# sebhaan/geobo

Hardware: AMD Instinct MI355X
Metric: voxels/sec posterior (mean+var) for 64^3 x 2-prop joint inversion; fp64 roofline % (higher is better)
Workload: dtype f64

## Files before the change

### geobo_amd/_lib.py

```python
import ctypes as C
import os

LIB_PATH = os.environ.get("GEOBO_HIP_LIB") or os.path.join(os.path.dirname(os.path.abspath(__file__)), "lib", "libgeobo_hip.so")

_dp = C.c_void_p
_i64 = C.c_int64
_f64 = C.c_double
_int = C.c_int
_sz = C.c_size_t

SIGNATURES = {
    "geobo_version": (_int, []),
    "geobo_pad_m": (_i64, [_i64]),
    "geobo_pad_n": (_i64, [_i64]),
    "geobo_k_block": (_int, [_int, _dp, _dp, _dp, _i64, _dp, _dp, _dp, _i64, _f64, _f64, _f64, _f64, _dp, _i64, _dp]),
    "geobo_k_block_f32": (_int, [_int, _dp, _dp, _dp, _i64, _dp, _dp, _dp, _i64, _f64, _f64, _f64, _f64, _dp, _i64, _dp]),
    "geobo_k_block_grid": (_int, [_int, _int, _int, _dp, _dp, _i64, _i64, _i64, _i64, _int, _dp, _i64, _dp]),
    "geobo_lattice_wbuild": (_int, [_i64, _int, _int, _int, _dp, _dp, _dp, _dp]),
    "geobo_lattice_wplanes": (_int, [_i64, _int, _int, _int, _dp, _dp, _dp, _dp]),
    "geobo_xz2d_fold_inv_strided": (_int, [_int, _i64, _int, _dp, _i64, _i64, _dp, _dp, _dp, _i64, _i64, _i64, _dp]),
    "geobo_xz2d_fold_inv_mul": (_int, [_int, _i64, _int, _dp, _i64, _dp, _i64, _dp, _dp, _dp, _i64, _i64, _i64, _dp]),
    "geobo_xz2d_fold_conv_fwd": (_int, [_int, _i64, _int, _dp, _i64, _dp, _i64, _dp, _i64, _dp, _dp, _dp, _i64, _i64, _dp]),
    "geobo_sumsq_accum": (_int, [_i64, _i64, _dp, _i64, _dp, _i64, _int, _dp, _i64, _dp]),
    "geobo_lamdot_z": (_int, [_i64, _int, _int, _int, _dp, _dp, _dp, _dp]),
    "geobo_centro_fill": (_int, [_dp, _i64, _i64, _i64, _dp]),
    "geobo_transpose": (_int, [_i64, _i64, _dp, _i64, _dp, _i64, _dp]),
    "geobo_mirror_rows": (_int, [_dp, _i64, _i64, _i64, _i64, _int, _dp]),
    "geobo_mirror_dev_ws_bytes": (_sz, []),
    "geobo_mirror_dev": (_int, [_dp, _i64, _dp, _i64, _i64, _int, _int, _dp, _dp, _sz, _dp]),
    "geobo_colgemv_ws_bytes": (_sz, [_i64, _i64]),
    "geobo_colgemv": (_int, [_i64, _i64, _dp, _i64, _dp, _dp, _dp, _sz, _dp]),
    "geobo_rowgemv": (_int, [_i64, _i64, _dp, _i64, _dp, _dp, _dp]),
    "geobo_convert": (_int, [_int, _dp, _i64, _dp, _i64, _i64, _i64, _dp]),
    "geobo_round_f32": (_int, [_dp, _i64, _dp]),
    "geobo_k_eval": (_int, [_int, _dp, _i64, _f64, _f64, _f64, _f64, _dp, _dp]),
    "geobo_a_sens": (_int, [_int, C.POINTER(_f64), _dp, _i64, _int, _int, _int, _dp, _dp, _dp, _f64, _f64, _dp, _i64, _dp]),
    "geobo_a_sens_slab": (_int, [_int, C.POINTER(_f64), _dp, _i64, _int, _int, _int, _dp, _dp, _dp, _f64, _f64, _int, _int, _dp, _i64, _i64, _dp]),
    "geobo_potential": (_int, [_int, C.POINTER(_f64), _dp, _dp, _dp, _i64, _dp, _dp]),
    "geobo_ak_fused": (_int, [_int, _dp, _i64, _i64, _i64, _dp, _dp, _dp, _i64, _i64, _f64, _f64, _f64, _f64, _dp, _i64, _dp]),
    "geobo_ak_points": (_int, [_int, _dp, _i64, _i64, _i64, _dp, _dp, _dp, _dp, _dp, _dp, _i64, _f64, _f64, _f64, _f64, _dp, _i64, _dp]),
    "geobo_cov_table": (_int, [_int, _int, _int, _int, _f64, _f64, _f64, _f64, _f64, _f64, _f64, _dp, _dp]),
    "geobo_ak_fused_grid": (_int, [_dp, _i64, _i64, _i64, _int, _int, _int, _dp, _i64, _i64, _dp, _i64, _dp]),
    "geobo_gemm_nt": (_int, [_i64, _i64, _i64, _f64, _dp, _i64, _dp, _i64, _f64, _dp, _i64, _int, _i64, _dp]),
    "geobo_tile_order": (_i64, [_int, _int, _int, _int, _int, _int, _int, C.POINTER(_int), _i64]),
    "geobo_gemm_map": (_int, [_int, _int, _int, _int, _int, _int, _int, _int, C.POINTER(_int)]),
    "geobo_gemm_nt_splitk": (_int, [_i64, _i64, _i64, _int, _dp, _i64, _dp, _i64, _dp, _i64, _int, _i64, _dp, _sz, _dp]),
    "geobo_gemm_nn": (_int, [_i64, _i64, _i64, _f64, _dp, _i64, _dp, _i64, _f64, _dp, _i64, _int, _int, _dp]),
    "geobo_gemm_batched": (_int, [_int, _i64, _i64, _i64, _f64, _dp, _i64, _i64, _dp, _i64, _i64, _f64, _dp, _i64, _i64, _i64, _i64, _int, _dp]),
    "geobo_gemm_fold_lamdot": (_int, [_i64, _i64, _i64, _dp, _i64, _dp, _i64, _i64, _dp, _int, _i64, _dp, _i64, _dp]),
    "geobo_gemm_fold": (_int, [_int, _int, _i64, _i64, _i64, _dp, _i64, _i64, _dp, _i64, _i64, _dp, _i64, _i64, _i64, _i64, _i64, _dp]),
# ... 111 lines not shown
```

### geobo_amd/csrc/reduce.hip

```cpp
#include <hip/hip_runtime.h>
#include <stdint.h>
#include "geobo_hip.h"

namespace {

typedef double v2d __attribute__((ext_vector_type(2)));

__global__ void __launch_bounds__(256) sumsq_accum_kernel(int64_t rows, int64_t n2, const double* __restrict__ a, int64_t lda,
                                                          const double* __restrict__ b, int64_t ldb, int slots, double* __restrict__ ss,
                                                          int64_t ld_ss) {
  const int64_t c2 = (int64_t)blockIdx.x * 256 + threadIdx.x;
  if (c2 >= n2) return;
  const int slot = blockIdx.y;
  v2d acc = *reinterpret_cast<const v2d*>(ss + slot * ld_ss + 2 * c2);
  if (b) {
    for (int64_t r = slot; r < rows; r += slots) {
      const v2d x = *reinterpret_cast<const v2d*>(a + r * lda + 2 * c2) + *reinterpret_cast<const v2d*>(b + r * ldb + 2 * c2);
      acc.x = __builtin_fma(x.x, x.x, acc.x);
      acc.y = __builtin_fma(x.y, x.y, acc.y);
    }
  } else {
    for (int64_t r = slot; r < rows; r += slots) {
      const v2d x = *reinterpret_cast<const v2d*>(a + r * lda + 2 * c2);
      acc.x = __builtin_fma(x.x, x.x, acc.x);
// ... 57 lines not shown
        v2d w;
        w.x = v.y;
        w.y = v.x;
        *reinterpret_cast<v2d*>(dst + (n - 2 - c)) = w;
      } else {
        dst[n - 2 - c] = v.y;
        dst[n - 1 - c] = v.x;
      }
    } else {
      dst[0] = src[c];
    }
  }
}

__global__ void __launch_bounds__(256) mirror_rows_kernel(double* __restrict__ X, int64_t ld, int64_t m, int64_t r0, int64_t nb, int nz2) {
  const int64_t e = (int64_t)blockIdx.x * 256 + threadIdx.x;
  if (e >= nb * nz2) return;
  const int64_t b = e / nz2;
  const int64_t se = (nb - 1 - b) * nz2 + (e - b * nz2);
  for (int64_t r = r0 + blockIdx.y; r < m; r += gridDim.y)
    reinterpret_cast<v2d*>(X + r * ld)[e] = reinterpret_cast<const v2d*>(X + (m - 1 - r) * ld)[se];
}

__device__ __forceinline__ double max_keep_nan(double m, double v) { return (v > m || v != v) ? v : m; }

constexpr int MIRROR_SLOTS_X = 4, MIRROR_SLOTS_Y = 256;

__global__ void __launch_bounds__(256) mirror_dev_kernel(const double* __restrict__ a, int64_t lda, const double* __restrict__ b, int64_t ldb,
                                                         int64_t rows, int nx, int nz2, double* __restrict__ part) {
  __shared__ double sh[2][4];
  double dev = 0.0, mx = 0.0;
  const int pairs = nx * nz2;
  for (int64_t r = blockIdx.y; r < rows; r += gridDim.y) {
    const v2d* pa = reinterpret_cast<const v2d*>(a + r * lda);
    const v2d* pb = reinterpret_cast<const v2d*>(b + (rows - 1 - r) * ldb);
    for (int e = blockIdx.x * 256 + threadIdx.x; e < pairs; e += gridDim.x * 256) {
      const int x = e / nz2;
      const v2d u = pa[e], w = pb[(nx - 1 - x) * nz2 + (e - x * nz2)];
      dev = max_keep_nan(max_keep_nan(dev, __builtin_fabs(u.x - w.x)), __builtin_fabs(u.y - w.y));
      mx = max_keep_nan(max_keep_nan(mx, __builtin_fabs(u.x)), __builtin_fabs(u.y));
      mx = max_keep_nan(max_keep_nan(mx, __builtin_fabs(w.x)), __builtin_fabs(w.y));
    }
  }
  for (int o = 32; o > 0; o >>= 1) {
    dev = max_keep_nan(dev, __shfl_xor(dev, o));
    mx = max_keep_nan(mx, __shfl_xor(mx, o));
// ... 54 lines not shown
                     rows, cols, src, lds, dst, ldd);
  return hipGetLastError() == hipSuccess ? GEOBO_OK : GEOBO_E_LAUNCH;
}

extern "C" int geobo_centro_fill(double* B, int64_t ld, int64_t n, int64_t r0, void* stream) {
  if (!B || ((uintptr_t)B & 15) || n < 0 || r0 < 0 || r0 > n || 2 * r0 < n || ld < n) return GEOBO_E_ARG;
  if (ld & 1) return GEOBO_E_ALIGN;
  if (r0 == n) return GEOBO_OK;
  const int64_t gy = n - r0 < 65535 ? n - r0 : 65535;
  hipLaunchKernelGGL(centro_fill_kernel, dim3((unsigned)(((n + 1) / 2 + 255) / 256), (unsigned)gy), dim3(256), 0, (hipStream_t)stream, B, ld, n, r0);
  return hipGetLastError() == hipSuccess ? GEOBO_OK : GEOBO_E_LAUNCH;
}

extern "C" int geobo_mirror_rows(double* X, int64_t ld, int64_t m, int64_t r0, int64_t nb, int nz, void* stream) {
  if (!X || m < 0 || r0 < 0 || r0 > m || 2 * r0 < m || nb <= 0 || nz <= 0 || nb * nz > ld) return GEOBO_E_ARG;
  if ((nz & 1) || (ld & 1) || ((uintptr_t)X & 15)) return GEOBO_E_ALIGN;
  if (r0 == m) return GEOBO_OK;
  const int64_t pairs = nb * (nz / 2), gy = m - r0 < 65535 ? m - r0 : 65535;
  hipLaunchKernelGGL(mirror_rows_kernel, dim3((unsigned)((pairs + 255) / 256), (unsigned)gy), dim3(256), 0, (hipStream_t)stream, X, ld, m, r0, nb,
                     nz / 2);
  return hipGetLastError() == hipSuccess ? GEOBO_OK : GEOBO_E_LAUNCH;
}

extern "C" size_t geobo_mirror_dev_ws_bytes(void) { return sizeof(double) * 2 * MIRROR_SLOTS_X * MIRROR_SLOTS_Y; }

extern "C" int geobo_mirror_dev(const double* a, int64_t lda, const double* b, int64_t ldb, int64_t rows, int nx, int nz, double* out2, void* ws,
                                size_t ws_bytes, void* stream) {
  if (!a || !b || !out2 || !ws || rows <= 0 || nx <= 0 || nz <= 0 || ws_bytes < geobo_mirror_dev_ws_bytes()) return GEOBO_E_ARG;
  if ((int64_t)nx * nz > lda || (int64_t)nx * nz > ldb || (int64_t)nx * nz >= (1LL << 31)) return GEOBO_E_ARG;
  if ((nz & 1) || (lda & 1) || (ldb & 1) || ((uintptr_t)a & 15) || ((uintptr_t)b & 15) || ((uintptr_t)ws & 15)) return GEOBO_E_ALIGN;
  const int pairs = nx * (nz / 2);
  const int gx = (pairs + 255) / 256 < MIRROR_SLOTS_X ? (pairs + 255) / 256 : MIRROR_SLOTS_X;
  const int gy = rows < MIRROR_SLOTS_Y ? (int)rows : MIRROR_SLOTS_Y;
  hipLaunchKernelGGL(mirror_dev_kernel, dim3(gx, gy), dim3(256), 0, (hipStream_t)stream, a, lda, b, ldb, rows, nx, nz / 2, (double*)ws);
  hipLaunchKernelGGL(mirror_dev_finish_kernel, dim3(1), dim3(256), 0, (hipStream_t)stream, (const double*)ws, gx * gy, out2);
  return hipGetLastError() == hipSuccess ? GEOBO_OK : GEOBO_E_LAUNCH;
}

extern "C" int geobo_rowgemv(int64_t m, int64_t n, const double* X, int64_t ld, const double* v, double* out, void* stream) {
  if (!X || !v || !out) return GEOBO_E_ARG;
  if (m <= 0 || n <= 0) return GEOBO_OK;
  if ((n & 1) || (ld & 1) || ld < n || ((uintptr_t)X & 15) || ((uintptr_t)v & 15)) return GEOBO_E_ALIGN;
  const int64_t nb = m < 256 * 16 ? m : 256 * 16;
  hipLaunchKernelGGL(rowgemv_kernel, dim3((unsigned)nb), dim3(256), 0, (hipStream_t)stream, m, n / 2, X, ld, v, out);
  return hipGetLastError() == hipSuccess ? GEOBO_OK : GEOBO_E_LAUNCH;
}
// ... 27 lines not shown
```

### geobo_amd/engine.py

```python
import math
import os
import time

import numpy as np
import torch

from . import geometry, hip
from .plan import COLUMN_FORM_MAX_BYTES, engine_options, feed_options, gram_gx_route, plan_route
from .columnform import ColumnExchangeMixin
from .rowform import RowFormMixin
from .operators import StreamedOperator
from .transposed import TransposedPosteriorMixin
from .information import SetStatisticsMixin
from .crossval import CrossValidationMixin
from .blocksupport import BlockSupportMixin
from .pointpred import PointPredictionMixin
from .resources import ResourceMixin
from .geobodies import GeobodyMixin
from .intercepts import InterceptMixin
from .append import AppendRowsMixin
from .reweight import ReweightMixin
from .step import Prior, Step
from .sharding import (EmulatedGroup, allreduce_sum_, assemble_columns, backend_of, exchange_blocks, exchange_blocks_finish,
                       exchange_blocks_start, gather_rows, gather_slices, shard_columns)

F64 = hip.F64


class _GramFeed:

    def __init__(self, gram, lams, S, store_all=True):
# ... 103 lines not shown
        s = settings
        self.nx, self.ny, self.nz = int(s.xNcube), int(s.yNcube), int(s.zNcube)
        self.N = self.nx * self.ny * self.nz
        self.N_pad = hip.pad_n(self.N)
        self.Ms = self.nx * self.ny
        self.Ms_pad = hip.pad_m(self.Ms)
        self.c0, self.c1 = shard_columns(self.N_pad, world, rank)
        self.nc = self.c1 - self.c0
        self._xyz = None
        self._A = {}
        self._ws = {}
        self._host = {}
        self._auto_denied = set()
        self._pending_exchange = None
        self.use_grid = self.nz >= 16 and self.nz % 2 == 0
        if method not in ("auto", "dense", "spectral"):
            raise ValueError("method must be 'auto', 'dense' or 'spectral'")
        self.method = method
        env = os.environ
        self.route = plan_route(self.nx, self.ny, self.nz, world=world, rank=rank, assembly=assembly, operators=operators, method=method,
                                env=env)
        self.options = engine_options(env)
        self.feed = feed_options(env)
        self.use_spectral = self.route.spectral
        if method == "spectral" and not self.use_spectral:
            raise ValueError("spectral method needs grid extents % 16 == 0 and column shards on y-slab boundaries")
        if self.route.operators == "streamed":
            self.streamed = True
        if self.route.note and self.N >= 32768:
            import warnings
            warnings.warn("geobo_amd route %s: %s" % (self.route.describe(), self.route.note), RuntimeWarning, stacklevel=3)
        self._spectral = None
        self._lattice_plan = None
        self._gram, self._lam, self._edgeV = None, {}, {}
        self._lamW, self._edgeVt = {}, {}
        self.aka_mirror_on = self.options.aka_mirror
        self.aka_mirror, self._mirror, self._mirror_meas = {}, {}, None
        self.z_spectrum_on = self.options.z_spectrum
        self.rows_static = self.route.rows
        self.exchange = self.route.exchange
        self._deny = {}
        self.step_route = None
        self._step = None
        self.last = None
        if self.streamed and not self.use_spectral:
            raise ValueError("streamed operators feed the spectral product: needs the spectral method's grid conditions")
# ... 357 lines not shown
                    hip.convert(out64, out)
            if Md:
                self._cov_rows(step.prior, 2, j, sel_t, self.c0, AK[off_d:off_d + Md, cols])
        return AK

    def _cov_rows(self, prior, i, j, rows_t, col0, out):
        ncv = min(out.shape[1], max(self.N - col0, 0))
        if ncv <= 0:
            return out
        if self.use_grid and col0 % 2 == 0:
            tab = prior.table(self, i, j)
            return hip.k_block_grid(tab, self.nx, self.ny, self.nz, rows_t, col0, out[:, :ncv])
        xyz = self.grid_points()
        rows = tuple(c[rows_t] for c in xyz)
        colc = tuple(c[col0:col0 + out.shape[1]] for c in xyz)
        return prior.k_block(self, i, j, rows, colc, out)

    def _assemble_AK_spectral(self, step, AK, A_g, A_m):
        sp, nc, props = self._spectral_product(), self.nc, step.props
        plane = self.nx * self.nz
        y0, y1 = self.c0 // plane, self.c1 // plane
        if self.exchange:
            return self._assemble_AK_spectral_exchange(step, AK)
        for s_, A in ((0, A_g), (1, A_m)):
            lams, outs, blocks = [], [], []
            for jj, j in enumerate(props):
                gen = sp.eigenvalues(step.prior.table(self, s_, j))
                step.gens[(s_, j)] = gen
                if step.sym and (s_, j) not in ((0, 0), (0, 1), (1, 1)):
                    continue
                lams.append(gen)
                blocks.append(j)
                outs.append(AK[s_ * self.Ms_pad:s_ * self.Ms_pad + self.Ms, jj * nc:(jj + 1) * nc])
            pooled = (isinstance(A, StreamedOperator) and A.lattice is not None and A.lattice.jy is not None and not self.f32
                      and sp.pool_applies())
            Mrun = step.mirror if (s_ == 1 and step.mirror) else self.Ms
            fl = sp.flops(Mrun, len(lams), y1 - y0, fwd_planes=sp.pool_planes(Mrun) if pooled else None)
            fv = sp.flops_valu(Mrun, len(lams), y1 - y0)
            feed = self._gram_feed(step, s_, blocks) if (y0, y1) == (0, self.ny) else None
            if feed is not None:
                fl += self._gram.flops_gx(Mrun * len(lams))

            def product_rows(gx, A=A, lams=lams, outs=outs, Mrun=Mrun, pooled=pooled):
                if not self.f32 and not isinstance(A, StreamedOperator):
                    return sp.product(A, Mrun, lams, [o[:Mrun] for o in outs], y0, y1, gx=gx)
                Rb = sp.R
                abuf = self._op_rows_buffer() if isinstance(A, StreamedOperator) else None
                scr = [self._workspace2d("ak_rows64_%d" % jj, Rb, nc) for jj in range(len(lams))] if self.f32 else None
                pool = sp.plane_pool(A.lattice, Mrun, A.lattice.jy, A.lattice.jx) if pooled else None
                for r0 in range(0, Mrun, Rb):
                    R = min(Rb, Mrun - r0)
                    if pool is not None:
                        src = pool.rows(r0)
                    elif abuf is not None and A.lattice is not None:
                        src = A.lattice.rows(r0)
                    else:
                        src = A.rows_into(abuf, r0, R) if abuf is not None else A[r0:r0 + R]
                    dst = [b[:R] for b in scr] if scr is not None else [o[r0:r0 + R] for o in outs]
                    sp.product(src, R, lams, dst, y0, y1, gx=gx and gx.at(r0))
                    if scr is not None:
                        for jj in range(len(lams)):
                            hip.convert(dst[jj], outs[jj][r0:r0 + R])
            self._timed("spectral_product", fl, lambda: product_rows(feed), valu=fv)
            if feed is not None and not feed.store_all:
                step.ak_fill.append(lambda fill=product_rows: fill(None))

    def _gram_feed(self, step, s_, blocks):
        gram, sp = self._gram, self._spectral_product()
        funcs = ("grav", "magn")
        if not (gram_gx_route(self.feed, self.route.family, step.sym, self.f32, self.world, self.exchange, self.nx, self.ny, self.nz, sp.forms)
                and gram is not None and gram.gx_applies() and sp.gx_applies() and all(j in (0, 1) and self._lam.get(funcs[j]) is not None for j in blocks)):
            return None
        S = [self._workspace("gram_S_%d%d" % (s_, j), (self.Ms * gram.Py * gram.Px,)) for j in blocks]
        for j, Sj in zip(blocks, S):
            step.gram_S[(s_, j)] = Sj
        return _GramFeed(gram, [self._lam[funcs[j]][1] for j in blocks], S, store_all=False)

    def _edge_spectrum(self, func, k, ycols):
        key = (func, k)
        hit = self._edgeV.get(key)
        if hit is None or hit[0] != ycols.data_ptr():
            hit = self._edgeV[key] = (ycols.data_ptr(), self._gram.edge_eigen(ycols))
        return hit[1]

    MIRROR_BOUND = 2.0 ** -48

    def _mirror_static(self, plan):
        return bool(self.aka_mirror_on and plan is not None and plan["rowmajor"] and self.route.family == "single" and self.world == 1
# ... 181 lines not shown
                    jj = props.index(j)
                    out[j * N:(j + 1) * N] = h[(k * P_c + jj) * N:(k * P_c + jj + 1) * N]
                else:
                    out[j * N:(j + 1) * N] = np.nan
            outs.append(out)
        return outs

    @_on_device
    def posterior(self, A_g, A_m, sel, y_g, y_m, y_d, lengths, crossweights, kernelfunc, gp_sigma, gp_amp=1.0,
                  props=(0, 1, 2), calclogl=True, want_mean_var=True, keep_K=False, potrf_schedule=None):
        props = tuple(props)
        assert 0 in props and 1 in props, "gravity and magnetic blocks are needed for AkA"
        sel = np.asarray(sel, dtype=np.int64)
        sel_t = torch.as_tensor(sel, device=self.device) if sel.size else None
        t = self._tick("start")
        scales = self._step_row_scale(sel)
        y = self._pad_y(y_g, y_m, y_d, hip.pad_m(2 * self.Ms_pad + len(sel)), None if scales is None else scales[1])
        if self.rows_static and not self._rows_denied and not self._rows_ok(A_g, A_m) and all(f in self._op_args for f in ("grav", "magn")):
            A_g, A_m = (self.operator(f, *self._op_args[f][:1], B=self._op_args[f][1], axes=self._op_args[f][2]) for f in ("grav", "magn"))
        step = self._step = self._new_step(Prior(kernelfunc, lengths, weight_matrix(crossweights), gp_amp), props, sel_t, gp_sigma,
                                           keep_signal=bool(keep_K), row_scale=scales, sym=not self.rows_static and self._sym_ok(A_g, A_m))
        M_pad = step.M_pad
        step.mirror = self._mirror_rows(step, A_m)
        for f, rec in self.aka_mirror.items():
            rec["taken"] = bool(f == "magn" and step.mirror)
        AK = self._assemble_AK(step, A_g, A_m)
        self.step_route = "rows" if step.rowpath else ("single" if step.sym else "columns")
        t = self._tick("ak_fused", t)
        AkA = self._assemble_AkA(step, AK, A_g, A_m)
        if self.aka_hook is not None:
            self.aka_hook(AkA)
        t = self._tick("aka", t)
        if self._potrf_ctx is None:
            self._potrf_ctx = hip.PotrfContext()
        Linv, info = self._timed("potrf_inv", 2.0 * M_pad ** 3 / 3.0, lambda: hip.potrf_inv(
            AkA, self._workspace("Linv", (M_pad, M_pad)), self._workspace("potrf_ws", (hip.potrf_ws_doubles(M_pad),)),
            ctx=self._potrf_ctx, schedule=potrf_schedule or self.options.potrf), alg=(2 * self.Ms + len(sel)) ** 3 * 2.0 / 3.0)
        L = AkA
        if scales is not None and scales[1].size:
            Linv.diagonal()[torch.as_tensor(scales[1], device=self.device)] = 0.0
        self._finish_exchange()
        u, stats = hip.trmv_stats(Linv, y, L)
        t = self._tick("cholesky", t)
        out = dict(info=0, M_pad=M_pad, lengths=[float(v) for v in lengths])

        def check_factor():
# ... 52 lines not shown
                    ws = self._workspace("post_ws", (hip.posterior_ws_doubles(M_pad, pw),))
                    parts = [hip.posterior_reduce(Linv, self._panel64("post_panel64", AK[:, cs:min(ncols, cs + pw)], cols=pw), u,
                                                  gp_amp * 1.0, ws, m_valid=Mv) for cs in range(0, ncols, pw)]
                    return torch.cat([p[0] for p in parts]), torch.cat([p[1] for p in parts])
                mu_l, var_l = self._timed("posterior_reduce", fl, panels, alg=(1.0 * Mu * Mu + 4.0 * Mu) * nv)
            one = self.world == 1 and self.N == self.N_pad
            mv = (mu_l, var_l, self.nc) if self.world == 1 else None
            N_ = len(props) * self.N
            hq = self._to_host_async(torch.cat([mu_l.reshape(-1)[:N_], var_l.reshape(-1)[:N_]]), 0) if one else None
            check_factor()
            t = self._tick("posterior", t)
            if one:
                out["mu"], out["var"] = self._results_to_host(mu_l, var_l, props, queued=hq)
            else:
                mu = assemble_columns(gather_slices(mu_l, len(props), self.N_pad, self.world, self.group), props, self.N,
                                      self.N_pad, self.world, to_host=self._to_host)
                var = assemble_columns(gather_slices(var_l, len(props), self.N_pad, self.world, self.group), props, self.N,
                                       self.N_pad, self.world, to_host=self._to_host)
                out["mu"], out["var"] = mu, var
            self._tick("d2h", t)
        whole = AK is not None and not step.sym
        self.last = _LastStep(L=L, Linv=Linv, u=u, AK=AK if whole else None, AK_partial=None if whole else AK, AK_complete=whole, props=props,
                              sel=sel, ops=(A_g, A_m), step=step, mv=mv, uu=out.get("uu"), logdet=out.get("logdet"))
        fills = list(step.ak_fill)
        if step.mirror and step.mirror < self.Ms:
            jj, nc, Msp, Mm = props.index(1), self.nc, self.Ms_pad, step.mirror
            fills.append(lambda: hip.mirror_rows(AK[Msp:Msp + self.Ms, jj * nc:jj * nc + self.N], self.Ms, Mm, self.nx * self.ny, self.nz))
        self.last.complete = _LastStep.chain(fills)
        return out

    def _derivative_gram(self, A_g, A_m, sel_t, prior, slot):
        step = self._new_step(prior, (0, 1, 2), sel_t, None, ak_slot="dK_AK", aka_slot=slot,
                              sym=not self.rows_static and self._sym_ok(A_g, A_m))
        return self._assemble_AkA(step, self._assemble_AK(step, A_g, A_m), A_g, A_m)

    @_on_device
    def logl_grad(self, A_g, A_m, sel, y_g, y_m, y_d, lengths, crossweights, kernelfunc, gp_sigma, gp_amp, directions,
                  potrf_schedule=None):
        if self.world > 1:
            raise ValueError("logl_grad runs on one rank (world = %d): the multi-rank gradient is not implemented" % self.world)
        if self.f32:
            raise ValueError("logl_grad needs the fp64 assembly (assembly='f32' keeps fp32 covariance tables)")
        directions = [np.asarray(d, dtype=float).reshape(3) for d in directions]
        if len(directions) > 3:
            raise ValueError("at most three length directions per evaluation")
        props = (0, 1, 2)
        r = self.posterior(A_g, A_m, sel, y_g, y_m, y_d, lengths, crossweights, kernelfunc, gp_sigma, gp_amp=gp_amp, props=props,
                           calclogl=True, want_mean_var=False, keep_K=True, potrf_schedule=potrf_schedule)
        W = weight_matrix(crossweights)
        Linv, u = self.last["Linv"], self.last["u"]
        M_pad = Linv.shape[0]
        sel = np.asarray(sel, dtype=np.int64)
# ... 115 lines not shown
```

### geobo_amd/hip.py

```python
import ctypes as C

import numpy as np
import torch

from . import _lib

F64 = torch.float64

KERNEL_IDS = {"d2": 0, "exp": 1, "exp_x": 2, "matern32": 3, "matern32_x": 4, "sparse": 5, "sparse_x": 6,
              "exp_dl": 7, "exp_x_dl1": 8, "exp_x_dl2": 9, "matern32_dl": 10, "matern32_x_dl1": 11, "matern32_x_dl2": 12,
              "sparse_dl": 13, "sparse_x_dl1": 14, "sparse_x_dl2": 15}
FUNC_IDS = {"grav": 0, "magn": 1}
from .plan import (PAD_M, PAD_N, SPECTRAL_AXIS_N, SPECTRAL_Y3T_NY, SPECTRAL_Y_NY, TOEPLITZ_ADD_NY, TOEPLITZ_NY, TOEPLITZ_Y2T_NY,
                   XZ2D_FOLD_N, XZ2D_SHAPES, YMUL_SHAPES)


def kernel_id(name, cross, deriv=None):
    if name not in ("exp", "matern32", "sparse"):
        raise ValueError("unknown kernelfunc %r (expected 'sparse', 'exp' or 'matern32')" % (name,))
    if deriv is None:
        return KERNEL_IDS[name + ("_x" if cross else "")]
    if isinstance(deriv, bool) or deriv not in (1, 2):
        raise ValueError("deriv must be None, 1 or 2, got %r" % (deriv,))
    if not cross:
# ... 173 lines not shown
def centro_fill(B, n, r0):
    lib = require_gpu()
    ld = _rowmajor(B, "B")
    assert B.shape[0] >= n and B.shape[1] >= n
    _lib.check(lib.geobo_centro_fill(_p(B), int(ld), int(n), int(r0), _stream()), "geobo_centro_fill")
    return B


def transpose(src, dst):
    lib = require_gpu()
    lds, ldd = _rowmajor(src, "src"), _rowmajor(dst, "dst")
    rows, cols = src.shape
    assert dst.shape[0] >= cols and dst.shape[1] >= rows
    _lib.check(lib.geobo_transpose(int(rows), int(cols), _p(src), int(lds), _p(dst), int(ldd), _stream()), "geobo_transpose")
    return dst


def mirror_rows(X, m, r0, nb, nz):
    lib = require_gpu()
    ld = _rowmajor(X, "X")
    assert X.shape[0] >= m and X.shape[1] >= nb * nz
    _lib.check(lib.geobo_mirror_rows(_p(X), int(ld), int(m), int(r0), int(nb), int(nz), _stream()), "geobo_mirror_rows")
    return X


def mirror_dev_ws_doubles():
    return require_gpu().geobo_mirror_dev_ws_bytes() // 8


def mirror_dev(a, b, rows, nx, nz, out=None, ws=None):
    lib = require_gpu()
    lda, ldb = _rowmajor(a, "a"), _rowmajor(b, "b")
    assert a.shape[0] >= rows and b.shape[0] >= rows
    nws = lib.geobo_mirror_dev_ws_bytes() // 8
    if ws is None:
        ws = torch.empty(nws, dtype=F64, device=a.device)
    if out is None:
        out = torch.empty(2, dtype=F64, device=a.device)
    _lib.check(lib.geobo_mirror_dev(_p(a), int(lda), _p(b), int(ldb), int(rows), int(nx), int(nz), _p(_chk(out, "out")), _p(_chk(ws, "ws")),
                                    ws.numel() * 8, _stream()), "geobo_mirror_dev")
    return out


def convert(src, dst):
    lib = require_gpu()
    assert src.shape == dst.shape and src.dim() == 2 and src.stride(1) == 1 and dst.stride(1) == 1
# ... 1073 lines not shown
```

### geobo_amd/plan.py

```python
from dataclasses import asdict, dataclass, make_dataclass

PAD_M, PAD_N = 256, 128
XZ2D_SHAPES = ((48, 64), (64, 64), (64, 32))
XZ2D_FOLD_N = (64,)
TOEPLITZ_NY = (16, 32, 48, 64, 80, 96, 112, 128)
SPECTRAL_AXIS_N = (80, 96, 112, 128)
SPECTRAL_Y_NY = (32, 48, 64, 80, 96, 112, 128)
TOEPLITZ_Y2T_NY = (32, 48, 64)
TOEPLITZ_ADD_NY = (80, 96, 112, 128)
SPECTRAL_Y3T_NY = (80, 96, 112, 128)
YMUL_SHAPES = ((128, 64),)
INTEGER_BASIS_N = (32, 64)
ROWS_MIN_VOXELS = 1 << 18
ROWS_MIN_PLANE = 96 * 96
ROWS_MIN_VOXELS_MID, ROWS_MIN_PLANE_MID = 3 << 17, 64 * 64
COLUMN_FORM_MAX_BYTES = 160 << 30
ROWS_MIN_VOXELS_FUSED = 1 << 17


SWITCHES = {"fused_xz": "GEOBO_SPECTRAL_FUSED_XZ",
            "fold": "GEOBO_XZ_FOLD",
            "quad": "GEOBO_XZ_QUAD",
            "dense_y": "GEOBO_SPECTRAL_DENSE_Y",
            "y_mfma": "GEOBO_Y_MFMA",
# ... 19 lines not shown
                  "row_chunk": ("GEOBO_ROW_CHUNK", 0, int),
                  "potrf": ("GEOBO_POTRF", "auto", lambda v: "dag" if v[:1] == "d" else "streams")}
EngineOptions = make_dataclass("EngineOptions", [(k, type(d)) for k, (_, d, _p) in ENGINE_OPTIONS.items()], frozen=True)


def engine_options(env=None):
    env = {} if env is None else env
    return EngineOptions(**{k: parse(env[var]) if var in env else default for k, (var, default, parse) in ENGINE_OPTIONS.items()})


FEED_OPTIONS = {"gram_gx": ("GEOBO_GRAM_GX", True, _on)}
FeedOptions = make_dataclass("FeedOptions", [(k, type(d)) for k, (_, d, _p) in FEED_OPTIONS.items()], frozen=True)


def feed_options(env=None):
    env = {} if env is None else env
    return FeedOptions(**{k: parse(env[var]) if var in env else default for k, (var, default, parse) in FEED_OPTIONS.items()})


def gram_gx_route(opts, family, sym, f32, world, exchange, nx, ny, nz, forms):
    return bool(opts.gram_gx and sym and family == "single" and not f32 and world == 1 and not exchange
                and nx == 64 and nz == 64 and ny % 2 == 0 and 4 <= ny <= 64
                and forms.xz == "fold" and forms.gram_x == "fold" and forms.y != "spectrum")


def half_integer(n):
    return n not in INTEGER_BASIS_N


@dataclass(frozen=True)
class Forms:
    xz: str
    x_axis4: bool
    y: str
    y_two_term: str
    y3t: bool
    y2s: bool
    fold: bool
    ss: str
    lattice_feed: bool
    plane_yx: str
    gram_x: str
    gram_y_axis4: bool
    zx: bool
    z_mul: bool
    ymul_slabs: tuple
# ... 137 lines not shown
```

### geobo_amd/step.py

```python
from dataclasses import dataclass, field


class Prior:

    def __init__(self, name, lengths, W, amp, deriv=None):
        self.name, self.lengths, self.W, self.amp = name, lengths, W, amp
        self.deriv = None if deriv is None else [float(v) for v in deriv]

    def terms(self, i, j):
        from .hip import kernel_id
        w, d = self.W[i][j], self.deriv
        if d is None:
            return [(kernel_id(self.name, i != j), w)]
        if i == j:
            return [(kernel_id(self.name, False, 1), w * d[j])]
        return [(kernel_id(self.name, True, 1), w * d[j]), (kernel_id(self.name, True, 2), w * d[i])]

    def table(self, eng, i, j):
        tabs = [eng._cov_table(kid, self.lengths[j], self.lengths[i], w, self.amp) for kid, w in self.terms(i, j)]
        for t in tabs[1:]:
            tabs[0].add_(t)
        return tabs[0]

    def k_block(self, eng, i, j, rows, cols, out):
# ... 23 lines not shown
        hip.ak_points(terms[0][0], A, xyz, q_xyz, self.lengths[j], self.lengths[s], terms[0][1], self.amp, out)
        for kid, w in terms[1:]:
            tmp = eng._workspace2d("dak_points_tmp", out.shape[0], out.shape[1])
            hip.ak_points(kid, A, xyz, q_xyz, self.lengths[j], self.lengths[s], w, self.amp, tmp)
            out.add_(tmp)
        return out


@dataclass
class Step:
    prior: Prior
    props: tuple
    sel_t: object
    Md: int
    M_pad: int
    noise: object = None
    ak_slot: str = "AK"
    aka_slot: str = "AkA"
    keep_signal: bool = False
    row_scale: object = None
    sym: bool = False
    rowpath: bool = False
    mirror: int = 0
    gens: dict = field(default_factory=dict)
    fullrows: dict = field(default_factory=dict)
    gram_S: dict = field(default_factory=dict)
    ak_fill: list = field(default_factory=list)
```

### geobo_amd/transposed.py

```python

import torch

from . import hip
from .operators import StreamedOperator

F64 = hip.F64


class TransposedPosteriorMixin:
    def _sym_ok(self, A_g, A_m):
        if not self._zpath_static_ok():
            return False
        return (self._gram is not None and self._gram.edge_supported() and self.Ms_pad == self.nx * self.ny
                and all(self._lam.get(f) is not None and self._lam[f][0] is A for f, A in (("grav", A_g), ("magn", A_m))))

    def _assemble_AkA_sym(self, step, AkA, AK, A_g, A_m):
        gram, pl, ny, Msp, nc = self._gram, self.nx * self.nz, self.ny, self.Ms_pad, self.nc
        Md, off_d, props = step.Md, 2 * self.Ms_pad, step.props
        lam = {0: self._lam["grav"][1], 1: self._lam["magn"][1]}
        ops = {0: A_g, 1: A_m}

        def edge_cols(sp_, k, iy):
            A = ops[sp_]
            if isinstance(A, StreamedOperator):
                return A.edge[:, k * pl:(k + 1) * pl] if A.lattice is not None else A.slab_into(self._workspace2d("op_slab", Msp, pl), iy, iy + 1)
            return A[:, iy * pl:(iy + 1) * pl]

        def rows_times_AT(X, nrows, sp_, out, S=None):
            if S is not None:
                gram.back_rows(S, nrows, out)
            else:
                gram.gram_rows(X, nrows, lam[sp_], out, 0, ny)
            for k, iy in enumerate((0, ny - 1)):
                gram.edge_rows(X[:, iy * pl:], nrows, self._edge_spectrum(("grav", "magn")[sp_], k, edge_cols(sp_, k, iy)), out)
        blk = lambda r0, j: AK[r0:, props.index(j) * nc:(props.index(j) + 1) * nc]

        Mm = step.mirror or self.Ms

        def run():
            rows_times_AT(blk(0, 0), self.Ms, 0, AkA[0:, 0:Msp], S.get((0, 0)))
            rows_times_AT(blk(0, 1), self.Ms, 1, AkA[0:, Msp:2 * Msp], S.get((0, 1)))
            rows_times_AT(blk(Msp, 1), Mm, 1, AkA[Msp:, Msp:2 * Msp], S.get((1, 1)))
            hip.transpose(AkA[:Msp, Msp:2 * Msp], AkA[Msp:2 * Msp, :Msp])
            if Md:
                rows_times_AT(blk(off_d, 0), Md, 0, AkA[off_d:, 0:Msp])
                rows_times_AT(blk(off_d, 1), Md, 1, AkA[off_d:, Msp:2 * Msp])
        S = step.gram_S
        nfed = sum(self.Ms if s_ == 0 else Mm for s_, _ in S)
        self._timed("aka_lattice", gram.flops(2 * self.Ms + Mm + 2 * Md - nfed, ny) + gram.flops_back(nfed), run)
        if step.mirror:
            self._timed("aka_centro_fill", 0.0, lambda: hip.centro_fill(AkA[Msp:Msp + self.Ms, Msp:Msp + self.Ms], self.Ms, (self.Ms + 1) // 2))
        return self._finish_AkA(step, AkA)

    def _zpath_static_ok(self):
        if not self.route.single or self.exchange:
            return False
        self._spectral_product()
        return True

    def _zpath_ok(self, step, AK):
        return (self._zpath_static_ok() and AK is not None and AK.dtype == F64
                and all((s_, j) in step.gens for s_ in (0, 1) for j in step.props))

    def _resident_operator(self, A, func):
        if not isinstance(A, StreamedOperator):
            return A
        R = self._workspace2d("A_" + func, self.Ms_pad, self.N_pad)
        xed, yed, zed = A.axes_dev
        hip.a_sens(A.func, A.Bv, A.locd, self.nx, self.ny, self.nz, xed, yed, zed, A.mul, A.div, R, plan=A.plan, ws=A.lws)
        return R

    def _lattice_Z(self, Lview, nrows, func, A, out, zx=False, edge=None):
# ... 199 lines not shown
```

### include/geobo_hip.h

```cpp
#ifndef GEOBO_HIP_H
#define GEOBO_HIP_H

#include <stddef.h>
#include <stdint.h>

#ifdef __cplusplus
extern "C" {
#endif

#define GEOBO_VERSION 213


#define GEOBO_PAD_M 256
#define GEOBO_PAD_N 128

enum { GEOBO_OK = 0, GEOBO_E_ARG = -1, GEOBO_E_ALIGN = -2, GEOBO_E_LAUNCH = -3, GEOBO_E_UNSUPPORTED = -4 };

enum {
  GEOBO_K_D2 = 0,
  GEOBO_K_EXP = 1,
  GEOBO_K_EXP_X = 2,
  GEOBO_K_MATERN32 = 3,
  GEOBO_K_MATERN32_X = 4,
  GEOBO_K_SPARSE = 5,
// ... 177 lines not shown
int geobo_spectral_y3t(int ny, int64_t C, int64_t plane, int64_t R, int nprop, const double* in_g, const double* in_m,
                       const double* const* tabs_g, const double* const* tabs_m, double* const* outs, const double* basis, void* stream);

int geobo_spectral_axis(int inverse, int n, int64_t C, int64_t plane_in, int64_t plane_out, int64_t item_in, int64_t item_out, int64_t items,
                        const double* in, double* out, const double* basis, int mask_ends, void* stream);

enum { GEOBO_POTRF_AUTO = 0, GEOBO_POTRF_STREAMS = 1, GEOBO_POTRF_DAG = 2 };
size_t geobo_potrf_ws_bytes(int64_t m);
int geobo_potrf_ctx_create(void** ctx);
int geobo_potrf_ctx_destroy(void* ctx);
int geobo_potrf_inv(int64_t m, double* A, int64_t ld, double* Linv, int64_t ldi, int* info, void* ws,
                    size_t ws_bytes, void* ctx, int schedule, void* stream);

int geobo_rowgemv(int64_t m, int64_t n, const double* X, int64_t ld, const double* v, double* out, void* stream);

int geobo_sumsq_accum(int64_t rows, int64_t n, const double* a, int64_t lda, const double* b, int64_t ldb, int slots, double* ss,
                      int64_t ld_ss, void* stream);

int geobo_lamdot_z(int64_t batch, int planes, int px, int nz, const double* D, const double* lam, double* out, void* stream);

int geobo_centro_fill(double* B, int64_t ld, int64_t n, int64_t r0, void* stream);
int geobo_transpose(int64_t rows, int64_t cols, const double* src, int64_t lds, double* dst, int64_t ldd, void* stream);
int geobo_mirror_rows(double* X, int64_t ld, int64_t m, int64_t r0, int64_t nb, int nz, void* stream);
size_t geobo_mirror_dev_ws_bytes(void);
int geobo_mirror_dev(const double* a, int64_t lda, const double* b, int64_t ldb, int64_t rows, int nx, int nz, double* out2, void* ws,
                     size_t ws_bytes, void* stream);

size_t geobo_posterior_ws_bytes(int64_t m, int64_t ncols);
int geobo_posterior_reduce(int64_t m, int64_t ncols, const double* Linv, int64_t ldi, const double* AK, int64_t ldak,
                           const double* u, double prior_var, double* mu, double* var, int64_t m_valid, void* ws,
                           size_t ws_bytes, void* stream);

size_t geobo_kinv_dot_ws_bytes(int64_t m, int T);
int geobo_kinv_dot(int64_t m, const double* Linv, int64_t ldl, const double* alpha, int T, const double* const* G, int64_t ldg,
                   const int64_t* seg, double* out, void* ws, size_t ws_bytes, void* stream);

int geobo_trmv_stats(int64_t m, const double* Linv, int64_t ldi, const double* y, const double* L, int64_t ld,
                     double* u, double* stats, void* stream);

int geobo_mfma_f64_peak(int blocks, int iters, double* out, void* stream);

int geobo_mfma_mix(int mode, int nv, int blocks, int iters, double* out, void* stream);

enum { GEOBO_RNG_PRIOR = 0, GEOBO_RNG_OBS = 1 };
#define GEOBO_FFT_INVERSE 1
#define GEOBO_FFT_IN_PAIRS 2
// ... 80 lines not shown
```

Measured before the change: 2.501 million.

## Compute grav-magn cross Gram block from mirrored magn rows instead of grav rows

Adds a route that computes the off-diagonal AK·Aᵀ cross block from the magnetic side. Only the mirror half of rows (Mm) goes through the interior Gram, and centro-symmetric fill, plane mirroring and a transpose complete the block. The AK products for the cross blocks the symmetric path needs are reorganised to match, and leftover blocks are deferred to the late fill. This replaces a full Ms-row Gram with an Mm-row one plus cheap copy kernels. It adds a new mirror_planes kernel and complexity around which AK blocks are filled when. It is enabled by default for 64³ grids.

```diff
diff --git a/geobo_amd/_lib.py b/geobo_amd/_lib.py
--- a/geobo_amd/_lib.py
+++ b/geobo_amd/_lib.py
@@ -26,6 +26,7 @@
     "geobo_centro_fill": (_int, [_dp, _i64, _i64, _i64, _dp]),
     "geobo_transpose": (_int, [_i64, _i64, _dp, _i64, _dp, _i64, _dp]),
     "geobo_mirror_rows": (_int, [_dp, _i64, _i64, _i64, _i64, _int, _dp]),
+    "geobo_mirror_planes": (_int, [_dp, _i64, _dp, _i64, _i64, _i64, _i64, _int, _int, _dp]),
     "geobo_mirror_dev_ws_bytes": (_sz, []),
     "geobo_mirror_dev": (_int, [_dp, _i64, _dp, _i64, _i64, _int, _int, _dp, _dp, _sz, _dp]),
     "geobo_colgemv_ws_bytes": (_sz, [_i64, _i64]),
diff --git a/geobo_amd/csrc/reduce.hip b/geobo_amd/csrc/reduce.hip
--- a/geobo_amd/csrc/reduce.hip
+++ b/geobo_amd/csrc/reduce.hip
@@ -103,6 +103,16 @@
     reinterpret_cast<v2d*>(X + r * ld)[e] = reinterpret_cast<const v2d*>(X + (m - 1 - r) * ld)[se];
 }
 
+__global__ void __launch_bounds__(256) mirror_planes_kernel(const double* __restrict__ src, int64_t lds, double* __restrict__ dst, int64_t ldd,
+                                                            int64_t m, int64_t r0, int64_t r1, int nx, int nz2) {
+  const int64_t e = (int64_t)blockIdx.x * 256 + threadIdx.x;
+  if (e >= (int64_t)nx * nz2) return;
+  const int64_t x = e / nz2;
+  const int64_t se = (nx - 1 - x) * nz2 + (e - x * nz2);
+  for (int64_t r = r0 + blockIdx.y; r < r1; r += gridDim.y)
+    reinterpret_cast<v2d*>(dst + (m - 1 - r) * ldd)[e] = reinterpret_cast<const v2d*>(src + r * lds)[se];
+}
+
 __device__ __forceinline__ double max_keep_nan(double m, double v) { return (v > m || v != v) ? v : m; }
 
 constexpr int MIRROR_SLOTS_X = 4, MIRROR_SLOTS_Y = 256;
@@ -203,6 +213,18 @@
   return hipGetLastError() == hipSuccess ? GEOBO_OK : GEOBO_E_LAUNCH;
 }
 
+extern "C" int geobo_mirror_planes(const double* src, int64_t lds, double* dst, int64_t ldd, int64_t m, int64_t r0, int64_t r1, int nx, int nz,
+                                   void* stream) {
+  if (!src || !dst || m < 0 || r0 < 0 || r0 > r1 || r1 > m || nx <= 0 || nz <= 0 || (int64_t)nx * nz > lds || (int64_t)nx * nz > ldd)
+    return GEOBO_E_ARG;
+  if ((nz & 1) || (lds & 1) || (ldd & 1) || ((uintptr_t)src & 15) || ((uintptr_t)dst & 15)) return GEOBO_E_ALIGN;
+  if (r0 == r1) return GEOBO_OK;
+  const int64_t pairs = (int64_t)nx * (nz / 2), gy = r1 - r0 < 65535 ? r1 - r0 : 65535;
+  hipLaunchKernelGGL(mirror_planes_kernel, dim3((unsigned)((pairs + 255) / 256), (unsigned)gy), dim3(256), 0, (hipStream_t)stream, src, lds, dst,
+                     ldd, m, r0, r1, nx, nz / 2);
+  return hipGetLastError() == hipSuccess ? GEOBO_OK : GEOBO_E_LAUNCH;
+}
+
 extern "C" size_t geobo_mirror_dev_ws_bytes(void) { return sizeof(double) * 2 * MIRROR_SLOTS_X * MIRROR_SLOTS_Y; }
 
 extern "C" int geobo_mirror_dev(const double* a, int64_t lda, const double* b, int64_t ldb, int64_t rows, int nx, int nz, double* out2, void* ws,
diff --git a/geobo_amd/engine.py b/geobo_amd/engine.py
--- a/geobo_amd/engine.py
+++ b/geobo_amd/engine.py
@@ -6,7 +6,7 @@
 import torch
 
 from . import geometry, hip
-from .plan import COLUMN_FORM_MAX_BYTES, engine_options, feed_options, gram_gx_route, plan_route
+from .plan import COLUMN_FORM_MAX_BYTES, cross_options, cross_rows_route, engine_options, feed_options, gram_gx_route, plan_route
 from .columnform import ColumnExchangeMixin
 from .rowform import RowFormMixin
 from .operators import StreamedOperator
@@ -156,6 +156,7 @@
                                 env=env)
         self.options = engine_options(env)
         self.feed = feed_options(env)
+        self.cross = cross_options(env)
         self.use_spectral = self.route.spectral
         if method == "spectral" and not self.use_spectral:
             raise ValueError("spectral method needs grid extents % 16 == 0 and column shards on y-slab boundaries")
@@ -559,16 +560,16 @@
         y0, y1 = self.c0 // plane, self.c1 // plane
         if self.exchange:
             return self._assemble_AK_spectral_exchange(step, AK)
+        kept = ((0, 0), (0, 1), (1, 1))
+        run = ((0, 0), (1, 0), (1, 1)) if step.cross_rows == "magn" else kept
         for s_, A in ((0, A_g), (1, A_m)):
-            lams, outs, blocks = [], [], []
+            gen_of, out_of = {}, {}
             for jj, j in enumerate(props):
-                gen = sp.eigenvalues(step.prior.table(self, s_, j))
-                step.gens[(s_, j)] = gen
-                if step.sym and (s_, j) not in ((0, 0), (0, 1), (1, 1)):
-                    continue
-                lams.append(gen)
-                blocks.append(j)
-                outs.append(AK[s_ * self.Ms_pad:s_ * self.Ms_pad + self.Ms, jj * nc:(jj + 1) * nc])
+                gen_of[j] = sp.eigenvalues(step.prior.table(self, s_, j))
+                step.gens[(s_, j)] = gen_of[j]
+                out_of[j] = AK[s_ * self.Ms_pad:s_ * self.Ms_pad + self.Ms, jj * nc:(jj + 1) * nc]
+            blocks = [j for j in props if not step.sym or (s_, j) in run]
+            lams, outs = [gen_of[j] for j in blocks], [out_of[j] for j in blocks]
             pooled = (isinstance(A, StreamedOperator) and A.lattice is not None and A.lattice.jy is not None and not self.f32
                       and sp.pool_applies())
             Mrun = step.mirror if (s_ == 1 and step.mirror) else self.Ms
@@ -599,8 +600,11 @@
                         for jj in range(len(lams)):
                             hip.convert(dst[jj], outs[jj][r0:r0 + R])
             self._timed("spectral_product", fl, lambda: product_rows(feed), valu=fv)
-            if feed is not None and not feed.store_all:
-                step.ak_fill.append(lambda fill=product_rows: fill(None))
+            whole = feed is None or feed.store_all
+            late = [j for j in props if (not step.sym or (s_, j) in kept) and not (whole and j in blocks)]
+            if late:
+                step.ak_fill.append(lambda fill=product_rows, lams=[gen_of[j] for j in late], outs=[out_of[j] for j in late]:
+                                    fill(None, lams=lams, outs=outs))
 
     def _gram_feed(self, step, s_, blocks):
         gram, sp = self._gram, self._spectral_product()
@@ -828,6 +832,7 @@
                                            keep_signal=bool(keep_K), row_scale=scales, sym=not self.rows_static and self._sym_ok(A_g, A_m))
         M_pad = step.M_pad
         step.mirror = self._mirror_rows(step, A_m)
+        step.cross_rows = "magn" if cross_rows_route(self.cross, step.sym, step.mirror, self.nx, self.ny, self.nz) else "grav"
         for f, rec in self.aka_mirror.items():
             rec["taken"] = bool(f == "magn" and step.mirror)
         AK = self._assemble_AK(step, A_g, A_m)
@@ -926,12 +931,15 @@
         whole = AK is not None and not step.sym
         self.last = _LastStep(L=L, Linv=Linv, u=u, AK=AK if whole else None, AK_partial=None if whole else AK, AK_complete=whole, props=props,
                               sel=sel, ops=(A_g, A_m), step=step, mv=mv, uu=out.get("uu"), logdet=out.get("logdet"))
+        self.last.complete = self._ak_completion(step, AK)
+        return out
+
+    def _ak_completion(self, step, AK):
         fills = list(step.ak_fill)
         if step.mirror and step.mirror < self.Ms:
-            jj, nc, Msp, Mm = props.index(1), self.nc, self.Ms_pad, step.mirror
+            jj, nc, Msp, Mm = step.props.index(1), self.nc, self.Ms_pad, step.mirror
             fills.append(lambda: hip.mirror_rows(AK[Msp:Msp + self.Ms, jj * nc:jj * nc + self.N], self.Ms, Mm, self.nx * self.ny, self.nz))
-        self.last.complete = _LastStep.chain(fills)
-        return out
+        return _LastStep.chain(fills)
 
     def _derivative_gram(self, A_g, A_m, sel_t, prior, slot):
         step = self._new_step(prior, (0, 1, 2), sel_t, None, ak_slot="dK_AK", aka_slot=slot,
diff --git a/geobo_amd/hip.py b/geobo_amd/hip.py
--- a/geobo_amd/hip.py
+++ b/geobo_amd/hip.py
@@ -219,6 +219,15 @@
     assert X.shape[0] >= m and X.shape[1] >= nb * nz
     _lib.check(lib.geobo_mirror_rows(_p(X), int(ld), int(m), int(r0), int(nb), int(nz), _stream()), "geobo_mirror_rows")
     return X
+
+
+def mirror_planes(src, dst, m, r0, r1, nx, nz):
+    lib = require_gpu()
+    lds, ldd = _rowmajor(src, "src"), _rowmajor(dst, "dst")
+    assert src.shape[0] >= r1 and dst.shape[0] >= m and src.shape[1] >= nx * nz and dst.shape[1] >= nx * nz
+    _lib.check(lib.geobo_mirror_planes(_p(src), int(lds), _p(dst), int(ldd), int(m), int(r0), int(r1), int(nx), int(nz), _stream()),
+               "geobo_mirror_planes")
+    return dst
 
 
 def mirror_dev_ws_doubles():
diff --git a/geobo_amd/plan.py b/geobo_amd/plan.py
--- a/geobo_amd/plan.py
+++ b/geobo_amd/plan.py
@@ -65,6 +65,30 @@
     return bool(opts.gram_gx and sym and family == "single" and not f32 and world == 1 and not exchange
                 and nx == 64 and nz == 64 and ny % 2 == 0 and 4 <= ny <= 64
                 and forms.xz == "fold" and forms.gram_x == "fold" and forms.y != "spectrum")
+
+
+CROSS_ROWS = ("auto", "magn", "grav")
+
+
+def _cross_rows(v):
+    if v not in CROSS_ROWS:
+        raise ValueError("GEOBO_CROSS_ROWS must be one of %s, got %r" % (", ".join(CROSS_ROWS), v))
+    return v
+
+
+CROSS_OPTIONS = {"cross_rows": ("GEOBO_CROSS_ROWS", "auto", _cross_rows)}
+CrossOptions = make_dataclass("CrossOptions", [(k, type(d)) for k, (_, d, _p) in CROSS_OPTIONS.items()], frozen=True)
+
+
+def cross_options(env=None):
+    env = {} if env is None else env
+    return CrossOptions(**{k: parse(env[var]) if var in env else default for k, (var, default, parse) in CROSS_OPTIONS.items()})
+
+
+def cross_rows_route(opts, sym, mirror_rows, nx, ny, nz):
+    if not (sym and mirror_rows) or opts.cross_rows == "grav":
+        return False
+    return opts.cross_rows == "magn" or nx == ny == nz == 64
 
 
 def half_integer(n):
diff --git a/geobo_amd/step.py b/geobo_amd/step.py
--- a/geobo_amd/step.py
+++ b/geobo_amd/step.py
@@ -69,6 +69,7 @@
     sym: bool = False
     rowpath: bool = False
     mirror: int = 0
+    cross_rows: str = "grav"
     gens: dict = field(default_factory=dict)
     fullrows: dict = field(default_factory=dict)
     gram_S: dict = field(default_factory=dict)
diff --git a/geobo_amd/transposed.py b/geobo_amd/transposed.py
--- a/geobo_amd/transposed.py
+++ b/geobo_amd/transposed.py
@@ -26,28 +26,48 @@
                 return A.edge[:, k * pl:(k + 1) * pl] if A.lattice is not None else A.slab_into(self._workspace2d("op_slab", Msp, pl), iy, iy + 1)
             return A[:, iy * pl:(iy + 1) * pl]
 
-        def rows_times_AT(X, nrows, sp_, out, S=None):
+        def interior(X, nrows, sp_, out, S=None):
             if S is not None:
                 gram.back_rows(S, nrows, out)
             else:
                 gram.gram_rows(X, nrows, lam[sp_], out, 0, ny)
+
+        def slabs(X, nrows, sp_, out):
             for k, iy in enumerate((0, ny - 1)):
                 gram.edge_rows(X[:, iy * pl:], nrows, self._edge_spectrum(("grav", "magn")[sp_], k, edge_cols(sp_, k, iy)), out)
+
+        def rows_times_AT(X, nrows, sp_, out, S=None):
+            interior(X, nrows, sp_, out, S)
+            slabs(X, nrows, sp_, out)
         blk = lambda r0, j: AK[r0:, props.index(j) * nc:(props.index(j) + 1) * nc]
 
         Mm = step.mirror or self.Ms
+        cross = step.cross_rows == "magn"
+
+        def cross_from_magn():
+            X, out, Ms = blk(Msp, 0), AkA[Msp:, 0:Msp], self.Ms
+            interior(X, Mm, 0, out, S.get((1, 0)))
+            hip.centro_fill(out[:Ms, :Ms], Ms, (Ms + 1) // 2)
+            for dst, src in ((0, ny - 1), (ny - 1, 0)):
+                hip.mirror_planes(X[:, src * pl:(src + 1) * pl], X[:, dst * pl:(dst + 1) * pl], Ms, 0, Ms - Mm, self.nx, self.nz)
+            slabs(X, Ms, 0, out)
+            hip.transpose(AkA[Msp:2 * Msp, :Msp], AkA[:Msp, Msp:2 * Msp])
 
         def run():
             rows_times_AT(blk(0, 0), self.Ms, 0, AkA[0:, 0:Msp], S.get((0, 0)))
-            rows_times_AT(blk(0, 1), self.Ms, 1, AkA[0:, Msp:2 * Msp], S.get((0, 1)))
+            if not cross:
+                rows_times_AT(blk(0, 1), self.Ms, 1, AkA[0:, Msp:2 * Msp], S.get((0, 1)))
             rows_times_AT(blk(Msp, 1), Mm, 1, AkA[Msp:, Msp:2 * Msp], S.get((1, 1)))
-            hip.transpose(AkA[:Msp, Msp:2 * Msp], AkA[Msp:2 * Msp, :Msp])
+            if cross:
+                cross_from_magn()
+            else:
+                hip.transpose(AkA[:Msp, Msp:2 * Msp], AkA[Msp:2 * Msp, :Msp])
             if Md:
                 rows_times_AT(blk(off_d, 0), Md, 0, AkA[off_d:, 0:Msp])
                 rows_times_AT(blk(off_d, 1), Md, 1, AkA[off_d:, Msp:2 * Msp])
         S = step.gram_S
         nfed = sum(self.Ms if s_ == 0 else Mm for s_, _ in S)
-        self._timed("aka_lattice", gram.flops(2 * self.Ms + Mm + 2 * Md - nfed, ny) + gram.flops_back(nfed), run)
+        self._timed("aka_lattice", gram.flops((self.Ms + 2 * Mm if cross else 2 * self.Ms + Mm) + 2 * Md - nfed, ny) + gram.flops_back(nfed), run)
         if step.mirror:
             self._timed("aka_centro_fill", 0.0, lambda: hip.centro_fill(AkA[Msp:Msp + self.Ms, Msp:Msp + self.Ms], self.Ms, (self.Ms + 1) // 2))
         return self._finish_AkA(step, AkA)
diff --git a/include/geobo_hip.h b/include/geobo_hip.h
--- a/include/geobo_hip.h
+++ b/include/geobo_hip.h
@@ -223,6 +223,8 @@
 int geobo_centro_fill(double* B, int64_t ld, int64_t n, int64_t r0, void* stream);
 int geobo_transpose(int64_t rows, int64_t cols, const double* src, int64_t lds, double* dst, int64_t ldd, void* stream);
 int geobo_mirror_rows(double* X, int64_t ld, int64_t m, int64_t r0, int64_t nb, int nz, void* stream);
+int geobo_mirror_planes(const double* src, int64_t lds, double* dst, int64_t ldd, int64_t m, int64_t r0, int64_t r1, int nx, int nz,
+                        void* stream);
 size_t geobo_mirror_dev_ws_bytes(void);
 int geobo_mirror_dev(const double* a, int64_t lda, const double* b, int64_t ldb, int64_t rows, int nx, int nz, double* out2, void* ws,
                      size_t ws_bytes, void* stream);
```

Result: faster. 2.656 million, median of 6 (+6.2%).
